# MuLabPKU/HD-PiSSA

Hardware: AMD Instinct MI355X
Metric: train tokens/sec (node) on the HD-PiSSA hot path, llama2-7b r16 (adapter probe fwd/bwd + Adam + dW aggregate + merge); dW merge+gather ms/step (higher is better)
Workload: dtype f32; 1 GPU; llama2-7b; model=llama2-7b, global_batch=16, seq_len=512, padding=per micro-batch to its longest sample (hp:190-201), micro_batches_per_rank=8, r_per_gpu=16, modules=224, exchange=gather, parallelism=dp1 (HD-PiSSA slices), x_layout=shared per projection group (q/k/v, gate/up)

## Files before the change

### hd-pissa_amd/csrc/hdp_probe.hip

```cpp
#include <chrono>
#include <cstdlib>
#include <cstring>
#include <mutex>
#include <vector>

#include "hdp_probe_int.h"

namespace hdp {

constexpr int kMaxGroup = 1024;
constexpr int kMaxSplit = 16;
constexpr int kP1Waves = 8;

static int p1_cols() {
  static const int v = [] { const char* e = getenv("HDP_P1_COLS"); return e ? atoi(e) : 128; }();
  return v;
}
static int p1_u() {
  static const int v = [] { const char* e = getenv("HDP_P1_U"); return e ? atoi(e) : 1; }();
  return v;
}
constexpr int kTC = 128;
constexpr int kNW = 256;

// ... 509 lines not shown
__device__ __forceinline__ void sweep_segment(const SweepDesc& d, int ct, int s0, int n, int64_t i0, int piece,
                                              const SweepArgs& sa, float* tile, float* red, int* flags, int wave,
                                              int lane) {
  constexpr bool PROJ = (MODE & kSwProj) != 0, OUTER = (MODE & kSwOuter) != 0;
  constexpr int rp = 16 * RB, r4 = rp / 4, ES = DT == HDP_F32 ? 4 : 2;
  const int li = lane & 15, g = lane >> 4;
  const int64_t T = d.T, N = d.N;
  const int64_t c = (int64_t)ct * kSwC + 64 * wave;
  const int64_t col = c + 4 * li;
  const int64_t colc = VEC ? (col < N ? col : N - 4) : col;
  const char* Zb = reinterpret_cast<const char*>(d.Z);

  constexpr bool SPLIT_F = DT == HDP_BF16 && MODE == kSwProj;
  constexpr bool X6 = K32 && DT == HDP_F32;
  constexpr bool K32P = K32 && MODE == kSwProj, K32O = K32 && MODE == kSwOuter;
  constexpr bool DL = K32P && DT == HDP_BF16 && !X6 && VEC;
  const int64_t cdl0 = c + 8 * g < N ? c + 8 * g : N - 8, cdl1 = c + 32 + 8 * g < N ? c + 32 + 8 * g : N - 8;
  f32x4 f[K32P ? 1 : 4][RB];
  bf16x4 fs[K32P ? 1 : 4][RB][3];
  bf16x8 fs8[K32P ? 2 : 1][RB][3];
  if constexpr (K32P) {
#pragma unroll
    for (int ch = 0; ch < 2; ++ch)
#pragma unroll
      for (int b = 0; b < RB; ++b) {
        const int j = 16 * b + li;
        const int64_t k = c + 32 * ch + 8 * g;
        float v[8];
#pragma unroll
        for (int e = 0; e < 8; ++e) v[e] = 0.f;
        const float* Fp = nullptr;
        int rows = d.r;
        if constexpr (FUSE) {
          Fp = b < d.nb ? d.Fb[b] : nullptr;
          rows = b < d.nb ? d.rbr[b] : 0;
        }
        const bool ok = FUSE ? (Fp != nullptr && li < rows) : (j < d.r);
        if (ok) {
          if (FUSE) Fp += (int64_t)li * N;
          if ((FUSE || d.f_rk) && N % 4 == 0 && k + 7 < N) {
            const float* P = FUSE ? Fp : d.F + (int64_t)j * N;
            const f32x4 a = gld4(P + k), bq = gld4(P + k + 4);
#pragma unroll
            for (int e = 0; e < 4; ++e) {
              v[e] = a[e];
              v[4 + e] = bq[e];
            }
          } else {
#pragma unroll
            for (int e = 0; e < 8; ++e)
              if (k + e < N)
                v[e] = FUSE ? gld1(Fp + k + e)
                            : d.f_rk ? gld1(d.F + (int64_t)j * N + k + e) : gld1(d.F + (k + e) * d.r + j);
          }
        }
        split8(v, fs8[ch][b][0], fs8[ch][b][1], fs8[ch][b][2]);
#pragma unroll
        for (int t = 0; t < 3; ++t) asm volatile("" : "+v"(fs8[ch][b][t]));
      }
  }
  if constexpr (PROJ && !K32P) {
#pragma unroll
    for (int s = 0; s < 4; ++s)
#pragma unroll
      for (int b = 0; b < RB; ++b) {
        const int j = 16 * b + li;
        const int64_t k = c + 16 * s + 4 * g;
        f32x4 v{0.f, 0.f, 0.f, 0.f};
        if constexpr (FUSE) {
          if (b < d.nb && li < d.rbr[b]) {
            const float* Fp = d.Fb[b] + (int64_t)li * N;
            if (N % 4 == 0 && k + 3 < N) {
              v = gld4(Fp + k);
            } else {
#pragma unroll
              for (int q = 0; q < 4; ++q)
                if (k + q < N) v[q] = gld1(Fp + k + q);
            }
          }
        } else if (j < d.r) {
          if (d.f_rk && N % 4 == 0 && k + 3 < N) {
            v = gld4(d.F + (int64_t)j * N + k);
          } else {
#pragma unroll
            for (int q = 0; q < 4; ++q)
              if (k + q < N) v[q] = d.f_rk ? gld1(d.F + (int64_t)j * N + k + q) : gld1(d.F + (k + q) * d.r + j);
          }
        }
        f[s][b] = v;
      }
    if constexpr (SPLIT_F) {
#pragma unroll
      for (int s = 0; s < 4; ++s)
#pragma unroll
        for (int b = 0; b < RB; ++b) {
          split3(f[s][b], fs[s][b][0], fs[s][b][1], fs[s][b][2]);
#pragma unroll
          for (int t = 0; t < 3; ++t) asm volatile("" : "+v"(fs[s][b][t]));
        }
    } else {
#pragma unroll
      for (int s = 0; s < 4; ++s)
#pragma unroll
        for (int b = 0; b < RB; ++b) asm volatile("" : "+v"(f[s][b]));
    }
  }
  bool hs_broken = false;
  f32x4 acc2[OUTER ? RB : 1][4];
#pragma unroll
  for (int b = 0; b < (OUTER ? RB : 1); ++b)
#pragma unroll
    for (int q = 0; q < 4; ++q) acc2[b][q] = f32x4{0.f, 0.f, 0.f, 0.f};

  constexpr bool DIST = PROJ && !FUSE && RB >= 4;
  int pend_i = -1, pend_s = 0;
  bool pend_tail = false;
  auto wait_ge = [&](const int* p, int target) {
    if (hs_broken) return;
    int it = 0;
    while (sa.spin < 0 || __hip_atomic_load(p, __ATOMIC_RELAXED, __HIP_MEMORY_SCOPE_WORKGROUP) < target) {
      if (it++ >= sa.spin) {
        hs_broken = true;
        if (lane == 0) {
          __hip_atomic_store(sa.err, 1, __ATOMIC_RELAXED, __HIP_MEMORY_SCOPE_SYSTEM);
          __hip_atomic_store(sa.errd, 1, __ATOMIC_RELAXED, __HIP_MEMORY_SCOPE_AGENT);
        }
        break;
      }
      __builtin_amdgcn_s_sleep(1);
    }
    asm volatile("" ::: "memory");
  };
  auto reduce_slice = [&](int pi, int ps, bool ptail) {
    if constexpr (DIST) {
      constexpr int NB = sw_nbuf<RB, FUSE>();
      const int pb = pi % NB, pr = pi / NB;
      wait_ge(flags + pb, kSwWaves * (pr + 1));
      const float* rs = red + pb * kSwWaves * 16 * rp;
      const int idx = 2 * lane;
      if (idx < 2 * rp) {
        const int row = 2 * wave + idx / rp, j = idx % rp;
        typedef float f32x2s __attribute__((ext_vector_type(2)));
        f32x2s acc{0.f, 0.f};
#pragma unroll
        for (int ww = 0; ww < kSwWaves; ++ww) acc += *reinterpret_cast<const f32x2s*>(rs + (ww * 16 + row) * rp + j);
        const int64_t t = 16 * (int64_t)ps + row;
        if (!ptail || t < T) *reinterpret_cast<HDP_GLOBAL f32x2s*>(gptr(d.slab_out + ((int64_t)ct * T + t) * rp + j)) = acc;
      }
      asm volatile("s_waitcnt lgkmcnt(0)" ::: "memory");
      if (lane == 0) (void)__hip_atomic_fetch_add(flags + NB + pb, 1, __ATOMIC_RELAXED, __HIP_MEMORY_SCOPE_WORKGROUP);
    }
  };

  auto compute = [&](const f32x4 (&z)[4], const float (&y)[4][RB], int s, int64_t i, bool tail) {
    if constexpr (OUTER) {
      if constexpr (DT == HDP_BF16) {
#pragma unroll
        for (int b = 0; b < RB; ++b) {
          if (FUSE && b >= d.nb) break;
          f32x4 yv;
#pragma unroll
          for (int p = 0; p < 4; ++p) yv[p] = (!tail || 16 * (int64_t)s + 4 * p + g < T) ? y[p][b] : 0.f;
          bf16x4 yh, ym, yl;
          split3(yv, yh, ym, yl);
#pragma unroll
          for (int q = 0; q < 4; ++q) {
            const bf16x4 zb{bf16_bits(z[0][q]), bf16_bits(z[1][q]), bf16_bits(z[2][q]), bf16_bits(z[3][q])};
            acc2[b][q] = mfma_bf16(yl, zb, acc2[b][q]);
            acc2[b][q] = mfma_bf16(ym, zb, acc2[b][q]);
            acc2[b][q] = mfma_bf16(yh, zb, acc2[b][q]);
          }
        }
      } else {
#pragma unroll
        for (int p = 0; p < 4; ++p) {
          const bool rok = !tail || 16 * (int64_t)s + 4 * p + g < T;
#pragma unroll
          for (int b = 0; b < RB; ++b) {
            if (FUSE && b >= d.nb) break;
            const float yv = rok ? y[p][b] : 0.f;
#pragma unroll
            for (int q = 0; q < 4; ++q) acc2[b][q] = __builtin_amdgcn_mfma_f32_16x16x4f32(yv, z[p][q], acc2[b][q], 0, 0, 0);
          }
        }
      }
    }
    if constexpr (PROJ) {
#pragma unroll
      for (int p = 0; p < (DL ? 0 : 4); ++p) *reinterpret_cast<f32x4*>(tile + (4 * p + g) * kTileLd + 4 * li) = z[p];
      f32x4 a0[RB], a1[RB];
#pragma unroll
      for (int b = 0; b < RB; ++b) a0[b] = a1[b] = f32x4{0.f, 0.f, 0.f, 0.f};
      if constexpr (K32P) {
#pragma unroll
        for (int ch = 0; ch < 2; ++ch) {
          f32x4 lo4{0.f, 0.f, 0.f, 0.f}, hi4{0.f, 0.f, 0.f, 0.f};
          if constexpr (!DL) {
            lo4 = *reinterpret_cast<const f32x4*>(tile + li * kTileLd + 32 * ch + 8 * g);
            hi4 = *reinterpret_cast<const f32x4*>(tile + li * kTileLd + 32 * ch + 8 * g + 4);
          }
          if constexpr (X6) {
            const float zv[8] = {lo4[0], lo4[1], lo4[2], lo4[3], hi4[0], hi4[1], hi4[2], hi4[3]};
            bf16x8 zs[3];
            split8p(zv, zs[0], zs[1], zs[2]);
#pragma unroll
            for (int b = 0; b < RB; ++b) {
              if (FUSE && b >= d.nb) break;
              f32x4& a = ch ? a1[b] : a0[b];
              a = mfma_x6(zs, fs8[ch][b], a);
            }
          } else {
            bf16x8 zb;
            if constexpr (DL) {
              zb = __builtin_bit_cast(bf16x8, z[ch]);
            } else {
#pragma unroll
              for (int e = 0; e < 4; ++e) {
                zb[e] = as_bf16(lo4[e]);
                zb[4 + e] = as_bf16(hi4[e]);
              }
            }
#pragma unroll
            for (int b = 0; b < RB; ++b) {
              if (FUSE && b >= d.nb) break;
              f32x4& a = ch ? a1[b] : a0[b];
              a = mfma32(zb, fs8[ch][b][2], a);
              a = mfma32(zb, fs8[ch][b][1], a);
              a = mfma32(zb, fs8[ch][b][0], a);
            }
          }
        }
      }
#pragma unroll
      for (int ss = 0; ss < (K32P ? 0 : 4); ++ss) {
        const f32x4 zf = *reinterpret_cast<const f32x4*>(tile + li * kTileLd + 16 * ss + 4 * g);
        if constexpr (SPLIT_F) {
          const bf16x4 zb{bf16_bits(zf[0]), bf16_bits(zf[1]), bf16_bits(zf[2]), bf16_bits(zf[3])};
#pragma unroll
          for (int b = 0; b < RB; ++b) {
            if (FUSE && b >= d.nb) break;
            f32x4& a = (ss & 1) ? a1[b] : a0[b];
            a = mfma_bf16(zb, fs[ss][b][2], a);
            a = mfma_bf16(zb, fs[ss][b][1], a);
            a = mfma_bf16(zb, fs[ss][b][0], a);
          }
        } else {
#pragma unroll
          for (int b = 0; b < RB; ++b) {
            if (FUSE && b >= d.nb) break;
#pragma unroll
            for (int q = 0; q < 4; ++q) {
              if (ss & 1) a1[b] = __builtin_amdgcn_mfma_f32_16x16x4f32(zf[q], f[ss][b][q], a1[b], 0, 0, 0);
              else a0[b] = __builtin_amdgcn_mfma_f32_16x16x4f32(zf[q], f[ss][b][q], a0[b], 0, 0, 0);
            }
          }
        }
      }
      HDP_MFMA_FENCE();
      constexpr int NBUF = sw_nbuf<RB, FUSE>();
      const int bsel = (int)(i % NBUF);
      const int round = (int)(i / NBUF);
      int* arrive = flags + bsel;
      int* done = flags + NBUF + bsel;
      if constexpr (DIST) {
        if (round > 0) wait_ge(done, kSwWaves * round);
        float* rb = red + (bsel * kSwWaves + wave) * 16 * rp;
#pragma unroll
        for (int b = 0; b < RB; ++b)
#pragma unroll
          for (int reg = 0; reg < 4; ++reg) rb[(4 * g + reg) * rp + 16 * b + li] = a0[b][reg] + a1[b][reg];
        asm volatile("s_waitcnt lgkmcnt(0)" ::: "memory");
        if (lane == 0) (void)__hip_atomic_fetch_add(arrive, 1, __ATOMIC_RELAXED, __HIP_MEMORY_SCOPE_WORKGROUP);
        if (pend_i >= 0) reduce_slice(pend_i, pend_s, pend_tail);
        pend_i = i;
        pend_s = s;
        pend_tail = tail;
      } else {
        if (round > 0 && !hs_broken) {
          int it = 0;
          while (sa.spin < 0 || __hip_atomic_load(done, __ATOMIC_RELAXED, __HIP_MEMORY_SCOPE_WORKGROUP) < round) {
            if (it++ >= sa.spin) {
              hs_broken = true;
              if (lane == 0) {
                __hip_atomic_store(sa.err, 1, __ATOMIC_RELAXED, __HIP_MEMORY_SCOPE_SYSTEM);
                __hip_atomic_store(sa.errd, 1, __ATOMIC_RELAXED, __HIP_MEMORY_SCOPE_AGENT);
              }
              break;
            }
            __builtin_amdgcn_s_sleep(1);
          }
          asm volatile("" ::: "memory");
        }
        float* rb = red + (bsel * kSwWaves + wave) * 16 * rp;
#pragma unroll
        for (int b = 0; b < RB; ++b) {
          if (FUSE && b >= d.nb) break;
#pragma unroll
          for (int reg = 0; reg < 4; ++reg) rb[(4 * g + reg) * rp + 16 * b + li] = a0[b][reg] + a1[b][reg];
        }
        asm volatile("s_waitcnt lgkmcnt(0)" ::: "memory");
        int old = 0;
        if (lane == 0) old = __hip_atomic_fetch_add(arrive, 1, __ATOMIC_RELAXED, __HIP_MEMORY_SCOPE_WORKGROUP);
        old = __builtin_amdgcn_readfirstlane(old);
        if (old == kSwWaves - 1) {
          asm volatile("s_waitcnt lgkmcnt(0)" ::: "memory");
          const float* rs = red + bsel * kSwWaves * 16 * rp;
          if constexpr (FUSE) {
#pragma unroll
            for (int b = 0; b < RB; ++b) {
              if (b >= d.nb) break;
              const int row = lane >> 2, jj = (lane & 3) * 4;
              f32x4 acc{0.f, 0.f, 0.f, 0.f};
#pragma unroll
              for (int ww = 0; ww < kSwWaves; ++ww)
                acc += *reinterpret_cast<const f32x4*>(rs + (ww * 16 + row) * rp + 16 * b + jj);
              const int64_t t = 16 * (int64_t)s + row;
              if (!tail || t < T) gst4(d.slab_b[b] + ((int64_t)ct * T + t) * d.rpm + jj, acc);
            }
          } else {
#pragma unroll
            for (int e0 = 0; e0 < 16 * r4; e0 += 64) {
              const int e = e0 + lane, row = e / r4, j = (e % r4) * 4;
              f32x4 acc{0.f, 0.f, 0.f, 0.f};
#pragma unroll
              for (int ww = 0; ww < kSwWaves; ++ww) acc += *reinterpret_cast<const f32x4*>(rs + (ww * 16 + row) * rp + j);
              const int64_t t = 16 * (int64_t)s + row;
              if (!tail || t < T) gst4(d.slab_out + ((int64_t)ct * T + t) * rp + j, acc);
            }
          }
          asm volatile("s_waitcnt lgkmcnt(0)" ::: "memory");
          if (lane == 0) {
            __hip_atomic_store(arrive, 0, __ATOMIC_RELAXED, __HIP_MEMORY_SCOPE_WORKGROUP);
            __hip_atomic_store(done, round + 1, __ATOMIC_RELAXED, __HIP_MEMORY_SCOPE_WORKGROUP);
          }
        }
      }
    }
  };

  auto pair = [&](const f32x4 (&zA)[4], const float (&yA)[4][RB], const f32x4 (&zB)[4], const float (&yB)[4][RB],
                  int s, bool vB, bool tail) {
    if constexpr (K32O && X6) {
      bf16x8 zs[4][3];
#pragma unroll
      for (int q = 0; q < 4; ++q) {
        const float zv[8] = {zA[0][q], zA[1][q], zA[2][q], zA[3][q],
                             vB ? zB[0][q] : 0.f, vB ? zB[1][q] : 0.f, vB ? zB[2][q] : 0.f, vB ? zB[3][q] : 0.f};
        split8p(zv, zs[q][0], zs[q][1], zs[q][2]);
      }
#pragma unroll
      for (int b = 0; b < RB; ++b) {
        if (FUSE && b >= d.nb) break;
        float yv[8];
#pragma unroll
        for (int p = 0; p < 4; ++p) {
          yv[p] = (!tail || 16 * (int64_t)s + 4 * p + g < T) ? yA[p][b] : 0.f;
          yv[4 + p] = vB ? yB[p][b] : 0.f;
        }
        bf16x8 ys[3];
        split8p(yv, ys[0], ys[1], ys[2]);
#pragma unroll
        for (int q = 0; q < 4; ++q) acc2[b][q] = mfma_x6(ys, zs[q], acc2[b][q]);
      }
    } else if constexpr (K32O) {
      bf16x8 zq[4];
#pragma unroll
      for (int q = 0; q < 4; ++q)
#pragma unroll
        for (int p = 0; p < 4; ++p) {
          zq[q][p] = as_bf16(zA[p][q]);
          zq[q][4 + p] = as_bf16(zB[p][q]);
        }
#pragma unroll
      for (int b = 0; b < RB; ++b) {
        if (FUSE && b >= d.nb) break;
        float yv[8];
#pragma unroll
        for (int p = 0; p < 4; ++p) {
          yv[p] = (!tail || 16 * (int64_t)s + 4 * p + g < T) ? yA[p][b] : 0.f;
          yv[4 + p] = vB ? yB[p][b] : 0.f;
        }
        bf16x8 yh, ym, yl;
        split8(yv, yh, ym, yl);
#pragma unroll
        for (int q = 0; q < 4; ++q) {
          acc2[b][q] = mfma32(yl, zq[q], acc2[b][q]);
          acc2[b][q] = mfma32(ym, zq[q], acc2[b][q]);
          acc2[b][q] = mfma32(yh, zq[q], acc2[b][q]);
        }
      }
    }
  };

  const int full_end = (int)min((int64_t)(s0 + n), T / 16);
  const int nfull = full_end > s0 ? full_end - s0 : 0;
  if (nfull > 0) {
    int64_t zo[4];
    int yo[4];
#pragma unroll
    for (int p = 0; p < 4; ++p) {
      zo[p] = ((16 * (int64_t)s0 + 4 * p + g) * N + colc) * ES;
      yo[p] = (16 * s0 + 4 * p + g) * d.yrs + li * d.yls;
    }
    const int64_t zstep = 16 * N * ES;
    int64_t zd = (16 * (int64_t)s0 + li) * N * ES;
    int lk = 0;
    auto load = [&](f32x4 (&z)[4], float (&y)[4][RB]) {
      __builtin_amdgcn_sched_barrier(0);
      if constexpr (DL) {
        typedef uint32_t u32x4d __attribute__((ext_vector_type(4)));
        z[0] = __builtin_bit_cast(f32x4, *reinterpret_cast<const HDP_GLOBAL u32x4d*>(gptr(Zb + zd + cdl0 * ES)));
        z[1] = __builtin_bit_cast(f32x4, *reinterpret_cast<const HDP_GLOBAL u32x4d*>(gptr(Zb + zd + cdl1 * ES)));
      }
#pragma unroll
      for (int p = 0; p < (DL ? 0 : 4); ++p) {
        if constexpr (VEC) {
          if constexpr (DT == HDP_F32)
            z[p] = load4_nt<DT>(Zb + zo[p], 0);
          else
            z[p] = load4<DT>(Zb + zo[p], 0);
        } else {
          const int64_t rowoff = zo[p] / ES - colc;
#pragma unroll
          for (int q = 0; q < 4; ++q) z[p][q] = load1<DT>(d.Z, rowoff + (col + q < N ? col + q : N - 1));
        }
        if constexpr (OUTER) {
          if constexpr (RB == 4) {
            const f32x4 v = gld4(d.y_in + yo[p]);
#pragma unroll
            for (int b = 0; b < RB; ++b) y[p][b] = v[b];
          } else if constexpr (RB == 2) {
            typedef float f32x2 __attribute__((ext_vector_type(2)));
            const f32x2 v = *reinterpret_cast<const HDP_GLOBAL f32x2*>(gptr(d.y_in + yo[p]));
            y[p][0] = v[0];
            y[p][1] = v[1];
          } else {
#pragma unroll
            for (int b = 0; b < RB; ++b) y[p][b] = gld1(d.y_in + yo[p] + b);
          }
        }
      }
      __builtin_amdgcn_sched_barrier(0);
      if (lk + 1 < nfull) {
        ++lk;
        zd += zstep;
#pragma unroll
        for (int p = 0; p < 4; ++p) {
          zo[p] += zstep;
          yo[p] += 16 * d.yrs;
        }
      }
    };
    if constexpr (K32O) {
      f32x4 za0[4], za1[4], zb0[4], zb1[4];
      float ya0[4][RB], ya1[4][RB], yb0[4][RB], yb1[4][RB];
      load(za0, ya0);
      load(za1, ya1);
      for (int k = 0; k < nfull; k += 4) {
        load(zb0, yb0);
        load(zb1, yb1);
        pair(za0, ya0, za1, ya1, s0 + k, k + 1 < nfull, false);
        load(za0, ya0);
        load(za1, ya1);
        if (k + 2 < nfull) pair(zb0, yb0, zb1, yb1, s0 + k + 2, k + 3 < nfull, false);
      }
    } else if constexpr (OCC == 1) {
      constexpr int NS = (DT == HDP_BF16 && MODE == kSwProj) ? kBfSets : 3;
      f32x4 zz[NS][4];
      float yy[NS][4][RB];
#pragma unroll
      for (int j = 0; j + 1 < NS; ++j) load(zz[j], yy[j]);
      for (int k = 0; k < nfull; k += NS) {
#pragma unroll
        for (int j = 0; j < NS; ++j) {
          load(zz[(j + NS - 1) % NS], yy[(j + NS - 1) % NS]);
          if (j == 0 || k + j < nfull) compute(zz[j], yy[j], s0 + k + j, i0 + k + j, false);
        }
      }
    } else {
      f32x4 z0[4], z1[4];
      float y0[4][RB], y1[4][RB];
      load(z0, y0);
      for (int k = 0; k < nfull; k += 2) {
        load(z1, y1);
        compute(z0, y0, s0 + k, i0 + k, false);
        load(z0, y0);
        if (k + 1 < nfull) compute(z1, y1, s0 + k + 1, i0 + k + 1, false);
      }
    }
  }
  if (nfull < n) {
    const int s = s0 + nfull;
    f32x4 z[4];
    float y[4][RB];
    if constexpr (DL) {
      typedef uint32_t u32x4d __attribute__((ext_vector_type(4)));
      int64_t row = 16 * (int64_t)s + li;
      row = row < T ? row : T - 1;
      z[0] = __builtin_bit_cast(f32x4, *reinterpret_cast<const HDP_GLOBAL u32x4d*>(gptr(Zb + (row * N + cdl0) * ES)));
      z[1] = __builtin_bit_cast(f32x4, *reinterpret_cast<const HDP_GLOBAL u32x4d*>(gptr(Zb + (row * N + cdl1) * ES)));
    }
#pragma unroll
    for (int p = 0; p < (DL ? 0 : 4); ++p) {
      int64_t row = 16 * (int64_t)s + 4 * p + g;
      row = row < T ? row : T - 1;
      if constexpr (VEC) {
        z[p] = load4<DT>(d.Z, row * N + colc);
      } else {
#pragma unroll
        for (int q = 0; q < 4; ++q) z[p][q] = load1<DT>(d.Z, row * N + (col + q < N ? col + q : N - 1));
      }
      if constexpr (OUTER) {
#pragma unroll
        for (int b = 0; b < RB; ++b) y[p][b] = gld1(d.y_in + row * d.yrs + li * d.yls + b);
      }
    }
    if constexpr (K32O)
      pair(z, y, z, y, s, false, true);
    else
      compute(z, y, s, i0 + nfull, true);
  }
  if constexpr (DIST) {
    if (pend_i >= 0) reduce_slice(pend_i, pend_s, pend_tail);
  }
  if constexpr (OUTER) {
    HDP_MFMA_FENCE();
    if (s0 == 0 && n == d.S) {
      if constexpr (FUSE) {
        if (col < N) sw_store_g_fuse(d, acc2, col, g, VEC);
      } else {
        if (col < N) sw_store_g<RB>(d, acc2, col, g, VEC);
      }
    } else if (FUSE && col < N) {
      const int64_t pofs = ((int64_t)ct * d.kmax + piece) * d.rpm * kSwC;
#pragma unroll
      for (int b = 0; b < RB; ++b) {
        if (b >= d.nb) break;
        float* base = d.part_b[b] + pofs;
        if (!d.part_t) {
#pragma unroll
          for (int reg = 0; reg < 4; ++reg)
            gst4(base + (4 * g + reg) * kSwC + 64 * wave + 4 * li,
                 f32x4{acc2[b][0][reg], acc2[b][1][reg], acc2[b][2][reg], acc2[b][3][reg]});
        } else {
#pragma unroll
          for (int q = 0; q < 4; ++q) gst4(base + (64 * wave + 4 * li + q) * d.rpm + 4 * g, acc2[b][q]);
        }
      }
    } else if (col < N) {
      float* base = d.part + ((int64_t)ct * d.kmax + piece) * rp * kSwC;
      if (!d.part_t) {
#pragma unroll
        for (int b = 0; b < RB; ++b)
#pragma unroll
          for (int reg = 0; reg < 4; ++reg)
            gst4(base + (16 * b + 4 * g + reg) * kSwC + 64 * wave + 4 * li,
                 f32x4{acc2[b][0][reg], acc2[b][1][reg], acc2[b][2][reg], acc2[b][3][reg]});
      } else {
#pragma unroll
        for (int b = 0; b < RB; ++b)
#pragma unroll
          for (int q = 0; q < 4; ++q)
            gst4(base + (64 * wave + 4 * li + q) * rp + 16 * b + 4 * g, acc2[b][q]);
      }
    }
  }
}

template <int DT, int RB, int MODE, bool VEC, int OCC, bool FUSE = false, bool K32 = false>
__global__ __launch_bounds__(512, OCC == 2 ? 4 : 2) void probe_sweep_kernel(SweepArgs sa) {
  extern __shared__ __attribute__((aligned(16))) float lds[];
  const int w = blockIdx.x;
  const int64_t nsteps = sa.bnd[w + 1] - sa.bnd[w];
  if (nsteps <= 0) return;
  const int lane = threadIdx.x & 63, wave = threadIdx.x >> 6;
  float* tile = lds + wave * 16 * kTileLd;
  float* red = lds + kSwWaves * 16 * kTileLd;
  int* flags = reinterpret_cast<int*>(red + sw_nbuf<RB, FUSE>() * kSwWaves * 16 * 16 * RB);
  if constexpr ((MODE & kSwProj) != 0) {
    if (threadIdx.x < 2 * sw_nbuf<RB, FUSE>()) flags[threadIdx.x] = 0;
    __syncthreads();
  }
  int m = sa.wst[4 * w], ct = sa.wst[4 * w + 1], s = sa.wst[4 * w + 2];
  int piece = sa.wst[4 * w + 3];
  for (int64_t done = 0; done < nsteps;) {
    const SweepDesc d = sa.d[m];
    const int n = (int)min((int64_t)(d.S - s), nsteps - done);
    sweep_segment<DT, RB, MODE, VEC, OCC, FUSE, K32>(d, ct, s, n, done, piece, sa, tile, red, flags, wave, lane);
    done += n;
    s = 0;
    piece = 0;
    if (++ct == d.nct) {
      ct = 0;
      ++m;
    }
  }
}

struct YReduceArgs {
  int n, rp;
  const YRedDesc* d;
};

__global__ __launch_bounds__(256) void probe_yreduce_kernel(YReduceArgs ya) {
  const YRedDesc d = ya.d[blockIdx.y];
  const int64_t f = (int64_t)blockIdx.x * 256 + threadIdx.x;
  const int64_t step4 = d.T * ya.rp / 4;
  if (f >= step4) return;
  const f32x4* src = reinterpret_cast<const f32x4*>(d.slab) + f;
  f32x4 acc{0.f, 0.f, 0.f, 0.f};
  for (int c0 = 0; c0 < d.nct; c0 += 8) {
    f32x4 v[8];
#pragma unroll
    for (int u = 0; u < 8; ++u) v[u] = c0 + u < d.nct ? gld4(reinterpret_cast<const float*>(src + (c0 + u) * step4)) : f32x4{0.f, 0.f, 0.f, 0.f};
#pragma unroll
    for (int u = 0; u < 8; ++u) acc += v[u];
  }
  const int rp = ya.rp;
  const int64_t e = 4 * f, t = e / rp;
  const int j0 = (int)(e % rp), b = j0 / 16, li0 = j0 % 16;
  float* dst = d.y + t * d.ys + b;
#pragma unroll
  for (int k = 0; k < 4; ++k) gst1(dst + (li0 + k) * d.sl, acc[k]);
}

struct SwFinishArgs {
  int n, rp;
  const FinDesc* d;
  const int* jobs;
  int bx;
};

template <int V>
__global__ __launch_bounds__(256) void probe_sweep_finish_kernel(SwFinishArgs fa) {
#pragma clang fp contract(off)
  typedef float vec __attribute__((ext_vector_type(V)));
  const int job = blockIdx.x / fa.bx;
  const FinDesc& dm = fa.d[fa.jobs[4 * job]];
  const int code = fa.jobs[4 * job + 1], ct = code >> 1;
  const bool sideA = (code & 1) == 0;
  const int r = dm.r;
  const int e = ((int)(blockIdx.x % fa.bx) * 256 + (int)threadIdx.x) * V;
  if (e >= r * kSwC) return;
  int nn, j;
  if (sideA) {
    j = e / kSwC;
    nn = e % kSwC;
  } else {
    nn = e / r;
    j = e % r;
  }
  const int64_t n = (int64_t)ct * kSwC + nn;
  if (n >= (sideA ? dm.in : dm.out)) return;
  const SwFinishSide& sd = sideA ? dm.sx : dm.sg;
  const int np = fa.jobs[4 * job + 2];
  const float* p = sd.part + (int64_t)ct * sd.kmax * fa.rp * kSwC + (sideA ? (int64_t)j * kSwC + nn : (int64_t)nn * fa.rp + j);
  const int64_t stride = (int64_t)fa.rp * kSwC;
  vec s0 = 0.f, s1 = 0.f;
  int k = 0;
  for (; k + 2 <= np; k += 2) {
    s0 += *reinterpret_cast<const HDP_GLOBAL vec*>(gptr(p + k * stride));
    s1 += *reinterpret_cast<const HDP_GLOBAL vec*>(gptr(p + (k + 1) * stride));
  }
  if (k < np) s0 += *reinterpret_cast<const HDP_GLOBAL vec*>(gptr(p + k * stride));
  const vec v = dm.scale * (s0 + s1);
  HDP_GLOBAL vec* gp = reinterpret_cast<HDP_GLOBAL vec*>(gptr(sideA ? dm.gA + (int64_t)j * dm.in + n : dm.gB + n * dm.ldb + j));
  *gp = dm.acc ? *gp + v : v;
}


static std::mutex g_err_mu;
static int* g_err_host = nullptr;
static int* g_err_dev = nullptr;
static int* g_err_local = nullptr;
int* probe_err_word() {
  std::lock_guard<std::mutex> lk(g_err_mu);
  if (!g_err_host) {
    void* h = nullptr;
    if (hipHostMalloc(&h, 256, hipHostMallocMapped) != hipSuccess) return nullptr;
    void* d = nullptr;
    if (hipHostGetDevicePointer(&d, h, 0) != hipSuccess) {
      (void)hipHostFree(h);
      return nullptr;
    }
    void* l = nullptr;
    if (hipMalloc(&l, 256) != hipSuccess || hipMemset(l, 0, 256) != hipSuccess) {
      (void)hipHostFree(h);
      return nullptr;
    }
    *reinterpret_cast<volatile int*>(h) = 0;
    g_err_host = reinterpret_cast<int*>(h);
    g_err_dev = reinterpret_cast<int*>(d);
    g_err_local = reinterpret_cast<int*>(l);
  }
  return g_err_dev;
}
int* probe_err_local() {
  std::lock_guard<std::mutex> lk(g_err_mu);
  return g_err_local;
}
const int* probe_err_device() { return probe_err_local(); }
int probe_err_read(int clear) {
  std::lock_guard<std::mutex> lk(g_err_mu);
  if (!g_err_host) return 0;
  volatile int* w = g_err_host;
  const int v = *w;
  if (clear && v != 0) {
    *w = 0;
    (void)hipMemset(g_err_local, 0, sizeof(int));
  }
  return v;
}
static int probe_spin() {
  const char* e = getenv("HDP_PROBE_SPIN");
  return e ? atoi(e) : (1 << 22);
}

struct Staging {
  void* host = nullptr;
  size_t cap = 0;
  hipEvent_t ev = nullptr;
  bool pending = false;
};
constexpr int kStageSlots = 64;
static std::mutex g_stage_mu;
static Staging g_stage[kStageSlots];
static int g_stage_next = 0;
static int64_t g_wait_ns = 0;

int probe_tables_upload(const std::vector<char>& blob, void* dst, hipStream_t st) {
  std::lock_guard<std::mutex> lk(g_stage_mu);
  Staging& s = g_stage[g_stage_next];
  g_stage_next = (g_stage_next + 1) % kStageSlots;
  if (s.pending) {
    if (hipEventQuery(s.ev) == hipErrorNotReady) {
      const auto t0 = std::chrono::steady_clock::now();
      HDP_CHECK_HIP(hipEventSynchronize(s.ev));
      g_wait_ns += std::chrono::duration_cast<std::chrono::nanoseconds>(std::chrono::steady_clock::now() - t0).count();
    }
    s.pending = false;
  }
  if (s.cap < blob.size()) {
    if (s.host) HDP_CHECK_HIP(hipHostFree(s.host));
    s.host = nullptr;
    s.cap = 0;
    const size_t sz = blob.size() * 2 > 65536 ? blob.size() * 2 : 65536;
    HDP_CHECK_HIP(hipHostMalloc(&s.host, sz, hipHostMallocDefault));
    s.cap = sz;
  }
  if (!s.ev) HDP_CHECK_HIP(hipEventCreateWithFlags(&s.ev, hipEventDisableTiming));
  memcpy(s.host, blob.data(), blob.size());
  HDP_CHECK_HIP(hipMemcpyAsync(dst, s.host, blob.size(), hipMemcpyHostToDevice, st));
  HDP_CHECK_HIP(hipEventRecord(s.ev, st));
  s.pending = true;
  return HDP_OK;
}

static void p1_split(int64_t K, int& ks, int& cols) {
  const int64_t span = (int64_t)kP1Waves * p1_cols();
  ks = (int)((K + span - 1) / span);
  int64_t c = (K + (int64_t)ks * kP1Waves - 1) / ((int64_t)ks * kP1Waves);
  cols = (int)((c + 15) / 16 * 16);
}

static bool use_sweep(int RB) {
  const char* e = getenv("HDP_PROBE_PATH");
  return RB <= 4 && !(e && e[0] == 's' && e[1] == 'p');
}

static bool slice_r(int r, int b_transposed) {
  const char* e = getenv("HDP_PROBE_R128");
  return r > 64 && r <= 128 && b_transposed && use_sweep(4) && !(e && e[0] == 's');
}
static int n_slices(int r) { return (r + 63) / 64; }

static ModPlan plan_module(int64_t T, int64_t in, int64_t out, int r) {
// ... 602 lines not shown
```

### hd-pissa_amd/csrc/hdp_sweep_plan.h

```cpp
#pragma once
#include <cstddef>
#include <cstdint>
#include <cstring>
#include <vector>

#include "hdp_probe_plan.h"

namespace hdp {

struct ProbeDesc {
  const void* X;
  const void* G;
  const float* A;
  const float* B;
  float* gA;
  float* gB;
  float* slabH;
  float* slabJ;
  float* partA;
  float* partB;
  float* yH;
  float* yJ;
  int64_t T, in, out;
  float scale;
  int r, b_t, accumulate;
  int ksh, ksj, kst;
  int colh, colj;
  int ldb;
};

struct HostGroup {
  int n = 0, rp = 16, RB = 1;
  std::vector<ProbeDesc> d;
};

constexpr int kSwWaves = 8;
constexpr int kSwC = 64 * kSwWaves;
constexpr int kSwMinSteps = 8;
constexpr int kSwMaxBlk = 4;

constexpr int kSwWeightA[kSwMaxBlk + 1] = {64, 64, 74, 88, 98};

struct SweepDesc {
  const void* Z;
  const float* F;
  float* slab_out;
  const float* y_in;
  float* part;
  int64_t T, N, pre;
  int r, f_rk, part_t, nct, S, kmax;
  float* g;
  float scale;
  int acc, ldb;
  int yrs, yls;
  int nb, rpm;
  const float* Fb[kSwMaxBlk];
  float* slab_b[kSwMaxBlk];
  float* part_b[kSwMaxBlk];
  float* gb[kSwMaxBlk];
  float sc[kSwMaxBlk];
  int rbr[kSwMaxBlk], accb[kSwMaxBlk];
};

struct YRedDesc {
  const float* slab;
  float* y;
  int64_t T;
  int nct, ys, sl, pad;
};

struct SwFinishSide {
  const float* part;
  int64_t pre;
  int S, kmax;
  int ph;
  int pad;
};
struct FinDesc {
  float* gA;
  float* gB;
  int in, out, r, acc;
  float scale;
  int ldb;
  SwFinishSide sx, sg;
};

static_assert(sizeof(SweepDesc) == 304, "SweepDesc layout");
static_assert(sizeof(YRedDesc) == 40, "YRedDesc layout");
static_assert(sizeof(SwFinishSide) == 32, "SwFinishSide layout");
static_assert(sizeof(FinDesc) == 104, "FinDesc layout");

constexpr size_t kTableFixed = 3 * 4096 * 5 * sizeof(int) + 8192;
constexpr size_t kTablePerModule = 3 * sizeof(SweepDesc) + 2 * sizeof(YRedDesc) + sizeof(FinDesc) + 64;

inline int rb_of(int r) {
  const int rb = (r + 15) / 16;
  return rb <= 1 ? 1 : rb <= 2 ? 2 : rb <= 4 ? 4 : 8;
}

struct ModPlan {
  int ksh, ksj, kst, colh, colj;
  size_t off_slabH, off_slabJ, off_partA, off_partB, off_yH, off_yJ, area, bytes;
};

inline size_t finish_jobs_bytes(int64_t in, int64_t out) {
  return (size_t)(((in + kSwC - 1) / kSwC + (out + kSwC - 1) / kSwC) * 16 + 255) / 256 * 256;
}

inline int sweep_kmax(int64_t T) { return (int)(((T + 15) / 16 + kSwMinSteps - 1) / kSwMinSteps) + 2; }

template <class Item>
inline size_t sweep_table_bytes(const Item* it, int n) {
  size_t b = kTableFixed + (size_t)n * kTablePerModule;
  for (int i = 0; i < n; ++i) b += finish_jobs_bytes(it[i].in, it[i].out);
  return b;
}

inline ModPlan plan_sweep_module(int64_t T, int64_t in, int64_t out, int r) {
  ModPlan p;
  const int RB = rb_of(r), rp = 16 * RB;
  size_t off = 0;
  auto take = [&](size_t n) { size_t o = off; off += (n * 4 + 255) / 256 * 256; return o; };
  p.ksh = (int)((in + kSwC - 1) / kSwC);
  p.ksj = (int)((out + kSwC - 1) / kSwC);
  p.colh = p.colj = 0;
  p.kst = sweep_kmax(T);
  const size_t T16 = (size_t)((T + 15) / 16) * 16;
  p.off_slabH = take((size_t)p.ksh * T16 * rp);
  p.off_slabJ = take((size_t)p.ksj * T16 * rp);
  p.off_partA = take((size_t)p.ksh * p.kst * rp * kSwC);
  p.off_partB = take((size_t)p.ksj * p.kst * rp * kSwC);
  const size_t yrow = RB <= 2 ? 64 : 2 * (size_t)rp;
  p.off_yH = take(T16 * yrow);
  p.off_yJ = take(T16 * yrow);
  p.area = off;
  p.bytes = off + kTablePerModule + kTableFixed + 256 + finish_jobs_bytes(in, out);
  return p;
}

inline void place_module(ProbeDesc& d, const ModPlan& p, char* area) {
  d.slabH = reinterpret_cast<float*>(area + p.off_slabH);
  d.slabJ = reinterpret_cast<float*>(area + p.off_slabJ);
  d.partA = reinterpret_cast<float*>(area + p.off_partA);
  d.partB = reinterpret_cast<float*>(area + p.off_partB);
  d.yH = reinterpret_cast<float*>(area + p.off_yH);
  d.yJ = reinterpret_cast<float*>(area + p.off_yJ);
  d.ksh = p.ksh;
  d.ksj = p.ksj;
  d.kst = p.kst;
  d.colh = p.colh;
  d.colj = p.colj;
}

struct SweepKnobs {
  bool share_x = true;
  bool balance = true;
  int k32 = 2;
  bool x6 = true;
};

struct SweepError {
  int code;
  const char* msg;
};
constexpr int kSweepEInval = 1;

inline std::vector<std::vector<int>> shared_x_sets(const HostGroup& ga, bool share_x) {
  std::vector<std::vector<int>> sets;
  const int n = ga.n;
  if (ga.RB > 2 || !share_x) return sets;
  for (int i = 0; i < n; ++i)
    if (!ga.d[i].b_t) return sets;
  std::vector<char> used(n, 0);
  for (int i = 0; i < n; ++i) {
    if (used[i]) continue;
    const ProbeDesc& p = ga.d[i];
    std::vector<int> cur{i};
    int64_t outs = p.out;
    for (int k = i + 1; k < n && (int)(cur.size() + 1) * ga.RB <= kSwMaxBlk; ++k) {
      const ProbeDesc& q = ga.d[k];
      if (!used[k] && q.X == p.X && q.T == p.T && q.in == p.in) {
        cur.push_back(k);
        outs += q.out;
      }
    }
    if (cur.size() < 2 || outs < p.in) continue;
    for (int k : cur) used[k] = 1;
    sets.push_back(cur);
  }
  return sets;
}

inline SweepDesc side_desc(const ProbeDesc& p, bool xs, int RB, int S) {
  const int rp = 16 * RB;
  SweepDesc d{};
  d.Z = xs ? p.X : p.G;
  d.F = xs ? p.A : p.B;
  d.slab_out = xs ? p.slabH : p.slabJ;
  d.y_in = xs ? p.yJ : p.yH;
  d.part = xs ? p.partA : p.partB;
  d.T = p.T;
  d.N = xs ? p.in : p.out;
  d.pre = 0;
  d.r = p.r;
  d.f_rk = xs ? 1 : p.b_t;
  d.part_t = xs ? 0 : 1;
  d.nct = xs ? p.ksh : p.ksj;
  d.S = S;
  d.kmax = p.kst;
  d.g = xs ? p.gA : p.gB;
  d.scale = p.scale;
  d.acc = p.accumulate;
  d.ldb = xs ? p.r : p.ldb;
  d.yrs = rp;
  d.yls = RB;
  d.nb = RB;
  d.rpm = rp;
  for (int b = 0; b < kSwMaxBlk; ++b) {
    const int rows = p.r - 16 * b;
    d.rbr[b] = b < RB ? (rows < 0 ? 0 : rows > 16 ? 16 : rows) : 0;
    d.Fb[b] = d.F + (int64_t)16 * b * d.N;
    d.slab_b[b] = d.slab_out + 16 * b;
    d.part_b[b] = d.part_t ? d.part + 16 * b : d.part + (int64_t)16 * b * kSwC;
    d.gb[b] = d.part_t ? d.g + 16 * b : d.g + (int64_t)16 * b * d.N;
    d.sc[b] = p.scale;
    d.accb[b] = p.accumulate;
  }
  return d;
}

struct SweepSides {
  bool split_b = false;
  bool fuse = false;
  bool v4 = true;
  bool weighted = false;
  std::vector<std::vector<int>> sets;
  std::vector<SweepDesc> sd[3];
  std::vector<YRedDesc> yd[2];
  std::vector<FinDesc> fd;
  int64_t U[3] = {0, 0, 0};
  int64_t yblk = 1;
  double bytes_ph[3] = {0, 0, 0}, flop_ph[3] = {0, 0, 0}, slab[2] = {0, 0};
};

inline void plan_sweep_sides(const HostGroup& ga, bool bf16, const SweepKnobs& kn, SweepSides& s) {
  const int n = ga.n, RB = ga.RB, rp = 16 * RB;
  const bool SPLIT_B = RB >= 4 && bf16;
  const int ES = bf16 ? 2 : 4;
  s.split_b = SPLIT_B;
  if (!SPLIT_B) s.sets = shared_x_sets(ga, kn.share_x);
  const std::vector<std::vector<int>>& sets = s.sets;
  const bool fuse = !sets.empty();
  s.fuse = fuse;
  s.weighted = fuse && !bf16 && kn.balance;
  std::vector<int> set_of(n, -1), blk0(n, 0);
  for (int k = 0; k < (int)sets.size(); ++k)
    for (int m = 0; m < (int)sets[k].size(); ++m) {
      set_of[sets[k][m]] = k;
      blk0[sets[k][m]] = m * RB;
    }
  std::vector<char> s1x(n);
  std::vector<int> at_c(n, -1), at_b(n, -1);
  auto add = [&](int ph, SweepDesc d) {
    d.pre = s.U[ph];
    s.U[ph] += (int64_t)d.nct * d.S;
    int rows = 0;
    for (int b = 0; b < d.nb && b < kSwMaxBlk; ++b) rows += d.rbr[b];
    s.bytes_ph[ph] += (double)ES * d.T * d.N;
    s.flop_ph[ph] += 2.0 * d.T * d.N * (fuse && (ph != 1) ? rows : d.r) * (ph == 1 && !SPLIT_B ? 2.0 : 1.0);
    s.sd[ph].push_back(d);
    return (int)s.sd[ph].size() - 1;
  };
  for (int k = 0; k < 2; ++k) s.yd[k].resize(n);
  s.fd.resize(n);
  for (int i = 0; i < n; ++i) {
    const ProbeDesc& p = ga.d[i];
    const int S = (int)((p.T + 15) / 16);
    const int si = set_of[i];
    s1x[i] = si >= 0 ? 1 : (p.in <= p.out);
    SweepDesc x = side_desc(p, true, RB, S), gg = side_desc(p, false, RB, S);
    if (si >= 0) {
      const ProbeDesc& lead = ga.d[sets[si][0]];
      gg.y_in = lead.yH + 16 * blk0[i];
      gg.yrs = 4 * 16;
      if (sets[si][0] == i) {
        SweepDesc fx = x;
        fx.nb = RB * (int)sets[si].size();
        fx.y_in = lead.yJ;
        fx.yrs = 4 * 16;
        fx.yls = 4;
        for (int m = 0; m < (int)sets[si].size(); ++m) {
          const SweepDesc xm = side_desc(ga.d[sets[si][m]], true, RB, S);
          for (int bb = 0; bb < RB; ++bb) {
            const int b = m * RB + bb;
            fx.Fb[b] = xm.Fb[bb];
            fx.rbr[b] = xm.rbr[bb];
            fx.slab_b[b] = xm.slab_b[bb];
            fx.part_b[b] = xm.part_b[bb];
            fx.gb[b] = xm.gb[bb];
            fx.sc[b] = xm.sc[bb];
            fx.accb[b] = xm.accb[bb];
          }
        }
        add(0, fx);
        at_c[i] = add(2, fx);
        for (int m : sets[si]) at_c[m] = at_c[i];
      }
      at_b[i] = add(1, gg);
    } else {
      const SweepDesc& d1 = s1x[i] ? x : gg;
      SweepDesc d2 = s1x[i] ? gg : x;
      SweepDesc d1c = d1;
      if (fuse) {
        d1c.yrs = 4 * 16;
        d1c.yls = 4;
      }
      add(0, d1);
      if (SPLIT_B) {
        add(1, d2);
        const int c1 = add(2, d1c);
        const int c2 = add(2, d2);
        at_c[i] = s1x[i] ? c1 : c2;
        at_b[i] = s1x[i] ? c2 : c1;
      } else {
        const int bi = add(1, d2);
        const int ci = add(2, d1c);
        at_c[i] = s1x[i] ? ci : bi;
        at_b[i] = s1x[i] ? bi : ci;
      }
    }
    if (si >= 0) {
      const ProbeDesc& lead = ga.d[sets[si][0]];
      s.yd[0][i] = YRedDesc{p.slabH, lead.yH + 16 * blk0[i], p.T, p.ksh, 4 * 16, RB, 0};
      s.yd[1][i] = YRedDesc{p.slabJ, lead.yJ + blk0[i], p.T, p.ksj, 4 * 16, 4, 0};
    } else {
      const SweepDesc& d1 = s1x[i] ? x : gg;
      const SweepDesc& d2 = s1x[i] ? gg : x;
      s.yd[0][i] = YRedDesc{d1.slab_out, s1x[i] ? p.yH : p.yJ, p.T, d1.nct, rp, RB, 0};
      s.yd[1][i] = YRedDesc{d2.slab_out, s1x[i] ? p.yJ : p.yH, p.T, d2.nct, fuse ? 4 * 16 : rp, fuse ? 4 : RB, 0};
    }
    const int64_t yb = (p.T * rp / 4 + 255) / 256;
    s.yblk = yb > s.yblk ? yb : s.yblk;
    s.fd[i] = FinDesc{p.gA, p.gB, (int)p.in, (int)p.out, p.r, p.accumulate, p.scale, p.ldb, {}, {}};
    s.v4 = s.v4 && p.r % 4 == 0 && p.ldb % 4 == 0 && p.in % 4 == 0 && (reinterpret_cast<uintptr_t>(p.gA) & 15) == 0 &&
           (reinterpret_cast<uintptr_t>(p.gB) & 15) == 0 && (reinterpret_cast<uintptr_t>(p.partA) & 15) == 0 &&
           (reinterpret_cast<uintptr_t>(p.partB) & 15) == 0;
  }
  for (int i = 0; i < n; ++i) {
    const ProbeDesc& p = ga.d[i];
    const bool x_in_c = SPLIT_B || s1x[i], g_in_c = SPLIT_B || !s1x[i];
    const SweepDesc& dx = s.sd[x_in_c ? 2 : 1][at_c[i]];
    const SweepDesc& dg = s.sd[g_in_c ? 2 : 1][at_b[i]];
    s.fd[i].sx = SwFinishSide{p.partA, dx.pre, dx.S, dx.kmax, x_in_c ? 1 : 0, 0};
    s.fd[i].sg = SwFinishSide{p.partB, dg.pre, dg.S, dg.kmax, g_in_c ? 1 : 0, 0};
    for (int k = 0; k < 2; ++k) s.slab[k] += 4.0 * p.T * rp * (s.yd[k][i].nct + 1);
  }
}

inline int phase_grid(int64_t U, int slots) {
  const int64_t cap = U / kSwMinSteps;
  return (int)(cap < 1 ? 1 : (cap < slots ? cap : slots));
}

inline int phase_ranges(const std::vector<SweepDesc>& d, int G, const int* weights, std::vector<int64_t>& bounds) {
  std::vector<PlanSide> sides(d.size());
  for (size_t i = 0; i < d.size(); ++i) {
    const int nb = d[i].nb < 1 ? 1 : d[i].nb > kSwMaxBlk ? kSwMaxBlk : d[i].nb;
    sides[i] = PlanSide{d[i].pre, d[i].nct, d[i].S, weights ? weights[nb] : 1};
  }
  return plan_ranges(sides, G, kSwMinSteps, bounds);
}

inline void phase_starts(const std::vector<SweepDesc>& d, const std::vector<int64_t>& bounds, int G, int* out,
                         int* bnd) {
  int m = 0;
  for (int w = 0; w <= G; ++w) bnd[w] = (int)bounds[w];
  for (int w = 0; w < G; ++w) {
    const int64_t lo = bounds[w];
    while (m + 1 < (int)d.size() && lo >= d[m + 1].pre) ++m;
    const int64_t rem = lo - d[m].pre;
    out[4 * w] = m;
    out[4 * w + 1] = (int)(rem / d[m].S);
    out[4 * w + 2] = (int)(rem % d[m].S);
    out[4 * w + 3] = w - plan_owner(bounds, lo - rem % d[m].S);
  }
}

struct SweepTables {
  int G[3] = {0, 0, 0};
  std::vector<int64_t> bounds[3];
  int njobs = 0;
  double pieces = 0;
  size_t o_sd[3] = {0, 0, 0}, o_w[3] = {0, 0, 0}, o_b[3] = {0, 0, 0}, o_y[2] = {0, 0}, o_f = 0, o_j = 0;
  std::vector<char> blob;
};

inline SweepError plan_sweep_tables(const HostGroup& ga, const SweepSides& s, const int slots[3], SweepTables& t) {
#define HDP_PLAN_CHECK(cond, text) \
  do {                             \
    if (!(cond)) return SweepError{kSweepEInval, text}; \
  } while (0)
  const int n = ga.n, rp = 16 * ga.RB;
  for (int ph = 0; ph < 3; ++ph) t.G[ph] = phase_grid(s.U[ph], slots[ph]);
  HDP_PLAN_CHECK(t.G[0] <= 4096 && t.G[1] <= 4096 && t.G[2] <= 4096, "probe sweep: grid above the table size");
  HDP_PLAN_CHECK(s.yblk < 65536 && n < 65536, "probe sweep: group too large");
  for (int ph = 0; ph < 3; ++ph) {
    HDP_PLAN_CHECK(s.U[ph] < (1ll << 31), "probe sweep: too many steps in one phase");
    t.G[ph] = phase_ranges(s.sd[ph], t.G[ph], s.weighted && ph == 0 ? kSwWeightA : nullptr, t.bounds[ph]);
    const int64_t least = s.U[ph] < kSwMinSteps ? s.U[ph] : kSwMinSteps;
    const std::vector<int64_t>& b = t.bounds[ph];
    bool ok = (int)b.size() == t.G[ph] + 1 && b[0] == 0 && b[t.G[ph]] == s.U[ph];
    for (int w = 0; ok && w < t.G[ph]; ++w) ok = b[w + 1] - b[w] >= least;
    HDP_PLAN_CHECK(ok, "probe sweep: a workgroup range below the minimum step count");
  }
  size_t off = 0;
  auto place = [&](size_t bytes) { size_t o = off; off += (bytes + 255) / 256 * 256; return o; };
  for (int ph = 0; ph < 3; ++ph) t.o_sd[ph] = place(sizeof(SweepDesc) * s.sd[ph].size());
  for (int ph = 0; ph < 3; ++ph) t.o_w[ph] = place(sizeof(int) * 4 * t.G[ph]);
  for (int ph = 0; ph < 3; ++ph) t.o_b[ph] = place(sizeof(int) * (t.G[ph] + 1));
  for (int k = 0; k < 2; ++k) t.o_y[k] = place(sizeof(YRedDesc) * n);
  t.o_f = place(sizeof(FinDesc) * n);
  std::vector<int> jobs;
  t.pieces = 0;
  for (int i = 0; i < n; ++i) {
    const ProbeDesc& p = ga.d[i];
    for (int side = 0; side < 2; ++side) {
      const SwFinishSide& fs = side == 0 ? s.fd[i].sx : s.fd[i].sg;
      const int nct = side == 0 ? p.ksh : p.ksj;
      const std::vector<int64_t>& b = t.bounds[fs.ph + 1];
      for (int ct = 0; ct < nct; ++ct) {
        const int64_t u0 = fs.pre + (int64_t)ct * fs.S;
        const int np = plan_owner(b, u0 + fs.S - 1) - plan_owner(b, u0) + 1;
        if (np > 1) {
          HDP_PLAN_CHECK(np <= fs.kmax, "probe sweep: a stripe has more pieces than its buffer holds");
          jobs.push_back(i);
          jobs.push_back(2 * ct + side);
          jobs.push_back(np);
          jobs.push_back(0);
          t.pieces += 4.0 * p.r * kSwC * ((double)np + (p.accumulate ? 2 : 1));
        }
      }
    }
  }
  t.njobs = (int)(jobs.size() / 4);
  HDP_PLAN_CHECK((int64_t)t.njobs * (rp * kSwC / 256) < (1ll << 31), "probe sweep: finish grid too large");
  t.o_j = place(sizeof(int) * jobs.size());
  HDP_PLAN_CHECK(off <= sweep_table_bytes(ga.d.data(), n), "probe sweep: descriptor tables exceed their space");
#undef HDP_PLAN_CHECK
  t.blob.resize(off);
  char* blob = t.blob.data();
  for (int ph = 0; ph < 3; ++ph) {
    if (!s.sd[ph].empty()) memcpy(blob + t.o_sd[ph], s.sd[ph].data(), sizeof(SweepDesc) * s.sd[ph].size());
    phase_starts(s.sd[ph], t.bounds[ph], t.G[ph], reinterpret_cast<int*>(blob + t.o_w[ph]),
                 reinterpret_cast<int*>(blob + t.o_b[ph]));
  }
  for (int k = 0; k < 2; ++k) memcpy(blob + t.o_y[k], s.yd[k].data(), sizeof(YRedDesc) * n);
  memcpy(blob + t.o_f, s.fd.data(), sizeof(FinDesc) * n);
  if (t.njobs) memcpy(blob + t.o_j, jobs.data(), sizeof(int) * jobs.size());
  return SweepError{0, nullptr};
}

}
```

Before: 195,600 tokens/s.

## Reorder probe y buffer into lane-swizzled layout for vectorized per-block loads

Changes the intermediate y buffer layout written by the y-reduction kernel so that each lane's four row values for one rank block sit contiguously. The sweep kernel can then load y with one 16-byte gld4 per block, replacing strided scalar or 2/4-wide loads across rows, and the tail path uses the same vector loads. The plan descriptors (yrs/yls/b0, offsets for grouped sets) are updated to match the new y_index mapping. The reduction store becomes a scattered scalar write, and the fused layout now uses kSwMaxBlk strides, which may pad or enlarge the buffer.

```diff
diff --git a/hd-pissa_amd/csrc/hdp_probe.hip b/hd-pissa_amd/csrc/hdp_probe.hip
--- a/hd-pissa_amd/csrc/hdp_probe.hip
+++ b/hd-pissa_amd/csrc/hdp_probe.hip
@@ -685,7 +685,7 @@
     }
   };
 
-  auto compute = [&](const f32x4 (&z)[4], const float (&y)[4][RB], int s, int64_t i, bool tail) {
+  auto compute = [&](const f32x4 (&z)[4], const f32x4 (&y)[RB], int s, int64_t i, bool tail) {
     if constexpr (OUTER) {
       if constexpr (DT == HDP_BF16) {
 #pragma unroll
@@ -693,7 +693,7 @@
           if (FUSE && b >= d.nb) break;
           f32x4 yv;
 #pragma unroll
-          for (int p = 0; p < 4; ++p) yv[p] = (!tail || 16 * (int64_t)s + 4 * p + g < T) ? y[p][b] : 0.f;
+          for (int p = 0; p < 4; ++p) yv[p] = (!tail || 16 * (int64_t)s + 4 * p + g < T) ? y[b][p] : 0.f;
           bf16x4 yh, ym, yl;
           split3(yv, yh, ym, yl);
 #pragma unroll
@@ -711,7 +711,7 @@
 #pragma unroll
           for (int b = 0; b < RB; ++b) {
             if (FUSE && b >= d.nb) break;
-            const float yv = rok ? y[p][b] : 0.f;
+            const float yv = rok ? y[b][p] : 0.f;
 #pragma unroll
             for (int q = 0; q < 4; ++q) acc2[b][q] = __builtin_amdgcn_mfma_f32_16x16x4f32(yv, z[p][q], acc2[b][q], 0, 0, 0);
           }
@@ -871,8 +871,8 @@
     }
   };
 
-  auto pair = [&](const f32x4 (&zA)[4], const float (&yA)[4][RB], const f32x4 (&zB)[4], const float (&yB)[4][RB],
-                  int s, bool vB, bool tail) {
+  auto pair = [&](const f32x4 (&zA)[4], const f32x4 (&yA)[RB], const f32x4 (&zB)[4], const f32x4 (&yB)[RB], int s,
+                  bool vB, bool tail) {
     if constexpr (K32O && X6) {
       bf16x8 zs[4][3];
 #pragma unroll
@@ -887,8 +887,8 @@
         float yv[8];
 #pragma unroll
         for (int p = 0; p < 4; ++p) {
-          yv[p] = (!tail || 16 * (int64_t)s + 4 * p + g < T) ? yA[p][b] : 0.f;
-          yv[4 + p] = vB ? yB[p][b] : 0.f;
+          yv[p] = (!tail || 16 * (int64_t)s + 4 * p + g < T) ? yA[b][p] : 0.f;
+          yv[4 + p] = vB ? yB[b][p] : 0.f;
         }
         bf16x8 ys[3];
         split8p(yv, ys[0], ys[1], ys[2]);
@@ -910,8 +910,8 @@
         float yv[8];
 #pragma unroll
         for (int p = 0; p < 4; ++p) {
-          yv[p] = (!tail || 16 * (int64_t)s + 4 * p + g < T) ? yA[p][b] : 0.f;
-          yv[4 + p] = vB ? yB[p][b] : 0.f;
+          yv[p] = (!tail || 16 * (int64_t)s + 4 * p + g < T) ? yA[b][p] : 0.f;
+          yv[4 + p] = vB ? yB[b][p] : 0.f;
         }
         bf16x8 yh, ym, yl;
         split8(yv, yh, ym, yl);
@@ -929,16 +929,13 @@
   const int nfull = full_end > s0 ? full_end - s0 : 0;
   if (nfull > 0) {
     int64_t zo[4];
-    int yo[4];
-#pragma unroll
-    for (int p = 0; p < 4; ++p) {
-      zo[p] = ((16 * (int64_t)s0 + 4 * p + g) * N + colc) * ES;
-      yo[p] = (16 * s0 + 4 * p + g) * d.yrs + li * d.yls;
-    }
+#pragma unroll
+    for (int p = 0; p < 4; ++p) zo[p] = ((16 * (int64_t)s0 + 4 * p + g) * N + colc) * ES;
+    int yo = ((4 * s0 + g) * d.yrs + li) * 4;
     const int64_t zstep = 16 * N * ES;
     int64_t zd = (16 * (int64_t)s0 + li) * N * ES;
     int lk = 0;
-    auto load = [&](f32x4 (&z)[4], float (&y)[4][RB]) {
+    auto load = [&](f32x4 (&z)[4], f32x4 (&y)[RB]) {
       __builtin_amdgcn_sched_barrier(0);
       if constexpr (DL) {
         typedef uint32_t u32x4d __attribute__((ext_vector_type(4)));
@@ -957,36 +954,23 @@
 #pragma unroll
           for (int q = 0; q < 4; ++q) z[p][q] = load1<DT>(d.Z, rowoff + (col + q < N ? col + q : N - 1));
         }
-        if constexpr (OUTER) {
-          if constexpr (RB == 4) {
-            const f32x4 v = gld4(d.y_in + yo[p]);
-#pragma unroll
-            for (int b = 0; b < RB; ++b) y[p][b] = v[b];
-          } else if constexpr (RB == 2) {
-            typedef float f32x2 __attribute__((ext_vector_type(2)));
-            const f32x2 v = *reinterpret_cast<const HDP_GLOBAL f32x2*>(gptr(d.y_in + yo[p]));
-            y[p][0] = v[0];
-            y[p][1] = v[1];
-          } else {
-#pragma unroll
-            for (int b = 0; b < RB; ++b) y[p][b] = gld1(d.y_in + yo[p] + b);
-          }
-        }
+      }
+      if constexpr (OUTER) {
+#pragma unroll
+        for (int b = 0; b < RB; ++b) y[b] = gld4(d.y_in + yo + 64 * b);
       }
       __builtin_amdgcn_sched_barrier(0);
       if (lk + 1 < nfull) {
         ++lk;
         zd += zstep;
 #pragma unroll
-        for (int p = 0; p < 4; ++p) {
-          zo[p] += zstep;
-          yo[p] += 16 * d.yrs;
-        }
+        for (int p = 0; p < 4; ++p) zo[p] += zstep;
+        yo += 16 * d.yrs;
       }
     };
     if constexpr (K32O) {
       f32x4 za0[4], za1[4], zb0[4], zb1[4];
-      float ya0[4][RB], ya1[4][RB], yb0[4][RB], yb1[4][RB];
+      f32x4 ya0[RB], ya1[RB], yb0[RB], yb1[RB];
       load(za0, ya0);
       load(za1, ya1);
       for (int k = 0; k < nfull; k += 4) {
@@ -1000,7 +984,7 @@
     } else if constexpr (OCC == 1) {
       constexpr int NS = (DT == HDP_BF16 && MODE == kSwProj) ? kBfSets : 3;
       f32x4 zz[NS][4];
-      float yy[NS][4][RB];
+      f32x4 yy[NS][RB];
 #pragma unroll
       for (int j = 0; j + 1 < NS; ++j) load(zz[j], yy[j]);
       for (int k = 0; k < nfull; k += NS) {
@@ -1012,7 +996,7 @@
       }
     } else {
       f32x4 z0[4], z1[4];
-      float y0[4][RB], y1[4][RB];
+      f32x4 y0[RB], y1[RB];
       load(z0, y0);
       for (int k = 0; k < nfull; k += 2) {
         load(z1, y1);
@@ -1025,7 +1009,7 @@
   if (nfull < n) {
     const int s = s0 + nfull;
     f32x4 z[4];
-    float y[4][RB];
+    f32x4 y[RB];
     if constexpr (DL) {
       typedef uint32_t u32x4d __attribute__((ext_vector_type(4)));
       int64_t row = 16 * (int64_t)s + li;
@@ -1043,10 +1027,10 @@
 #pragma unroll
         for (int q = 0; q < 4; ++q) z[p][q] = load1<DT>(d.Z, row * N + (col + q < N ? col + q : N - 1));
       }
-      if constexpr (OUTER) {
-#pragma unroll
-        for (int b = 0; b < RB; ++b) y[p][b] = gld1(d.y_in + row * d.yrs + li * d.yls + b);
-      }
+    }
+    if constexpr (OUTER) {
+#pragma unroll
+      for (int b = 0; b < RB; ++b) y[b] = gld4(d.y_in + ((4 * s + g) * d.yrs + li) * 4 + 64 * b);
     }
     if constexpr (K32O)
       pair(z, y, z, y, s, false, true);
@@ -1151,10 +1135,9 @@
   }
   const int rp = ya.rp;
   const int64_t e = 4 * f, t = e / rp;
-  const int j0 = (int)(e % rp), b = j0 / 16, li0 = j0 % 16;
-  float* dst = d.y + t * d.ys + b;
-#pragma unroll
-  for (int k = 0; k < 4; ++k) gst1(dst + (li0 + k) * d.sl, acc[k]);
+  const int j0 = (int)(e % rp), b = d.b0 + j0 / 16, li0 = j0 % 16;
+#pragma unroll
+  for (int k = 0; k < 4; ++k) gst1(d.y + y_index(t, b, li0 + k, d.sl), acc[k]);
 }
 
 struct SwFinishArgs {
diff --git a/hd-pissa_amd/csrc/hdp_sweep_plan.h b/hd-pissa_amd/csrc/hdp_sweep_plan.h
--- a/hd-pissa_amd/csrc/hdp_sweep_plan.h
+++ b/hd-pissa_amd/csrc/hdp_sweep_plan.h
@@ -62,11 +62,15 @@
   int rbr[kSwMaxBlk], accb[kSwMaxBlk];
 };
 
+constexpr int64_t y_index(int64_t t, int b, int li, int nb) {
+  return ((((t / 16 * 4 + t % 4) * nb + b) * 16 + li) * 4) + t % 16 / 4;
+}
+
 struct YRedDesc {
   const float* slab;
   float* y;
   int64_t T;
-  int nct, ys, sl, pad;
+  int nct, ys, sl, b0;
 };
 
 struct SwFinishSide {
@@ -276,19 +280,19 @@
   for (int i = 0; i < n; ++i) {
     const ProbeDesc& p = ga.d[i];
     const int S = (int)((p.T + 15) / 16);
+    const int64_t T16 = 16 * (int64_t)S;
     const int si = set_of[i];
     s1x[i] = si >= 0 ? 1 : (p.in <= p.out);
     SweepDesc x = side_desc(p, true, RB, S), gg = side_desc(p, false, RB, S);
     if (si >= 0) {
       const ProbeDesc& lead = ga.d[sets[si][0]];
-      gg.y_in = lead.yH + 16 * blk0[i];
-      gg.yrs = 4 * 16;
+      gg.y_in = lead.yH + (int64_t)blk0[i] * 16 * T16;
       if (sets[si][0] == i) {
         SweepDesc fx = x;
         fx.nb = RB * (int)sets[si].size();
         fx.y_in = lead.yJ;
-        fx.yrs = 4 * 16;
-        fx.yls = 4;
+        fx.yrs = 16 * kSwMaxBlk;
+        fx.yls = kSwMaxBlk;
         for (int m = 0; m < (int)sets[si].size(); ++m) {
           const SweepDesc xm = side_desc(ga.d[sets[si][m]], true, RB, S);
           for (int bb = 0; bb < RB; ++bb) {
@@ -312,8 +316,8 @@
       SweepDesc d2 = s1x[i] ? gg : x;
       SweepDesc d1c = d1;
       if (fuse) {
-        d1c.yrs = 4 * 16;
-        d1c.yls = 4;
+        d1c.yrs = 16 * kSwMaxBlk;
+        d1c.yls = kSwMaxBlk;
       }
       add(0, d1);
       if (SPLIT_B) {
@@ -331,13 +335,13 @@
     }
     if (si >= 0) {
       const ProbeDesc& lead = ga.d[sets[si][0]];
-      s.yd[0][i] = YRedDesc{p.slabH, lead.yH + 16 * blk0[i], p.T, p.ksh, 4 * 16, RB, 0};
-      s.yd[1][i] = YRedDesc{p.slabJ, lead.yJ + blk0[i], p.T, p.ksj, 4 * 16, 4, 0};
+      s.yd[0][i] = YRedDesc{p.slabH, lead.yH + (int64_t)blk0[i] * 16 * T16, p.T, p.ksh, rp, RB, 0};
+      s.yd[1][i] = YRedDesc{p.slabJ, lead.yJ, p.T, p.ksj, 16 * kSwMaxBlk, kSwMaxBlk, blk0[i]};
     } else {
       const SweepDesc& d1 = s1x[i] ? x : gg;
       const SweepDesc& d2 = s1x[i] ? gg : x;
       s.yd[0][i] = YRedDesc{d1.slab_out, s1x[i] ? p.yH : p.yJ, p.T, d1.nct, rp, RB, 0};
-      s.yd[1][i] = YRedDesc{d2.slab_out, s1x[i] ? p.yJ : p.yH, p.T, d2.nct, fuse ? 4 * 16 : rp, fuse ? 4 : RB, 0};
+      s.yd[1][i] = YRedDesc{d2.slab_out, s1x[i] ? p.yJ : p.yH, p.T, d2.nct, fuse ? 16 * kSwMaxBlk : rp, fuse ? kSwMaxBlk : RB, 0};
     }
     const int64_t yb = (p.T * rp / 4 + 255) / 256;
     s.yblk = yb > s.yblk ? yb : s.yblk;
```

Result: no change. 197,500 tokens/s, median of 6 (+1.0%).
